# qimao7213/SInDSLAM

Measured on AMD Instinct MI355X. Metric: DynaDetect+ORB frame-pairs/sec at 640x480; mask IoU vs CPU ref, higher is better.
Workload: dtype f32

## Files before the change

include/sind_hip.h:

```cpp
#ifndef SIND_HIP_H
#define SIND_HIP_H
#include <stddef.h>
#include <stdint.h>
#ifdef __cplusplus
extern "C" {
#endif

#define SIND_OK 0
#define SIND_E_ARG (-1)
#define SIND_E_HIP (-2)
#define SIND_E_ALLOC (-3)
#define SIND_E_STATE (-4)
#define SIND_E_CAPACITY (-5)

const char* sind_last_error(void);
int sind_device_count(int* count);

typedef struct sind_flow sind_flow;
int sind_flow_create(int fw, int fh, int max_batch, int device, sind_flow** out);
int sind_flow_destroy(sind_flow* f);
int sind_flow_levels(sind_flow* f, int* widths, int* heights, int cap);
int sind_flow_deepflow(sind_flow* f, const uint8_t* i0, const uint8_t* i1, int B, float* u, float* v);
int sind_flow_refine(sind_flow* f, const uint8_t* i0, const uint8_t* i1, int B, float* u, float* v);
int sind_flow_varref_f32(sind_flow* f, const float* i0, const float* i1, int w, int h, int B, float* u, float* v,
                         int fixed_point_iters, int sor_iters, float alpha, float delta, float gamma, float omega);
int sind_flow_deepflow_dev(sind_flow* f, const uint8_t* i0, const uint8_t* i1, int B, float* u, float* v);
int sind_flow_refine_dev(sind_flow* f, const uint8_t* i0, const uint8_t* i1, int B, float* u, float* v);
int sind_flow_sync(sind_flow* f);
int sind_flow_set_max_levels(sind_flow* f, int n);
int sind_flow_set_coarse_chain(sind_flow* f, int on);
int sind_flow_set_latency_tiles(sind_flow* f, int on);
int sind_flow_set_level_up(sind_flow* f, int on);
int sind_flow_set_sor(sind_flow* f, int mode, int fuse, int tile_w);
int sind_flow_set_sor_tiled(sind_flow* f, int mode, int fuse, int tile_w, int tile_h);
int sind_flow_set_solver_workgroups(sind_flow* f, int cap);
int sind_flow_set_wave_solver(sind_flow* f, int on, int target_items, int bands);
int sind_flow_wave_layout(int w, int h, int B, int target_items, int bands, int out[4]);
int sind_flow_sor_plan(int mode, int fuse, int tile_w, int tile_h, int wave, int stream_min_b, int latency_tiles, int coarse_chain, int w, int h, int B, int total, int* out, int cap);
int sind_flow_set_coef_kernel(sind_flow* f, int variant);
int sind_flow_timer_begin(sind_flow* f);
int sind_flow_timer_end(sind_flow* f, float* milliseconds);

typedef struct sind_orb sind_orb;
typedef struct sind_keypoint { float x, y, size, angle, response; int octave, class_id; } sind_keypoint;
int sind_orb_create(int nfeatures, float scale_factor, int nlevels, int ini_th_fast, int min_th_fast, int device, sind_orb** out);
int sind_orb_destroy(sind_orb* o);
int sind_orb_reserve(sind_orb* o, int width, int height, int max_batch);
int sind_orb_extract(sind_orb* o, const uint8_t* gray, int width, int height, int stride, const uint8_t* mask_or_null, int mask_stride,
                     sind_keypoint* kps, int cap, int* n, uint8_t* desc );
int sind_orb_extract_batch(sind_orb* o, const uint8_t* gray, int width, int height, int B, const uint8_t* masks_or_null,
                           sind_keypoint* kps, int cap, int* n, uint8_t* desc);
int sind_orb_tables(sind_orb* o, float* scale, float* inv_scale, float* sigma2, float* inv_sigma2, int* features_per_level, int* umax16);
int sind_orb_pyramid(sind_orb* o, int frame, int level, uint8_t* out, int* w, int* h);
int sind_orb_debug_fast(sind_orb* o, int frame, int level, float* xyr, int cap);
int sind_orb_debug_selected(sind_orb* o, int frame, sind_keypoint* kps, int cap, uint8_t* desc);
int sind_orb_debug_blurred(sind_orb* o, int frame, int level, uint8_t* out, int* w, int* h);

typedef struct sind_dyna sind_dyna;
int sind_dyna_create(int width, int height, float fx, float fy, float cx, float cy, float depth_scale, int device, sind_dyna** out);
int sind_dyna_destroy(sind_dyna* d);
int sind_dyna_set_flow_max_levels(sind_dyna* d, int n);
int sind_dyna_timing(sind_dyna* d, double ms12[12], int reset);
int sind_dyna_timing_fine(sind_dyna* d, double ms40[40], int reset);
int sind_dyna_set_debug(sind_dyna* d, int on);
int sind_dyna_set_overlap(sind_dyna* d, int on);
int sind_dyna_prime(sind_dyna* d, const uint8_t* bgr_last, const uint8_t* bgr_lastlast, int stride);
int sind_dyna_detect(sind_dyna* d, const uint8_t* bgr, int bgr_stride, const uint16_t* depth, int depth_stride,
                     uint8_t* dyna_out, uint8_t* label_out, int n_img);
int sind_dyna_dilate15(sind_dyna* d, uint8_t* dyna_inout);
int sind_dyna_debug(sind_dyna* d, float* flow_deep, float* flow_refined, float* flow_full, double* H9, float* thr5, int* hist256,
                    uint8_t* mask_low, uint8_t* mask_high, uint8_t* kmeans_label, float* centers36, uint8_t* occ1, uint8_t* occ2,
                    uint8_t* total_area, uint8_t* grad_edge, uint8_t* plane_contours, int* info3);

int sind_debug_seqsum(const float* x, int n, int device, float* out);
int sind_debug_set_kmeans_fused_max(int n);
int sind_debug_set_kmeans_fused_min_batch(int b);
int sind_debug_coef_math_scan(int device, int exp_lo, int exp_hi, const float numer[3], unsigned long long out[2]);
int sind_debug_rcp_scan(int device, int exp_lo, int exp_hi, unsigned long long out[3]);
int sind_debug_div_scan(int device, unsigned long long counts[3], int* max_exp, unsigned long long by_exp[124]);

int sind_debug_flow_thresholds(const int* hist, int n, int width, int height, int variant, int device, int* res, double* mu1);
int sind_debug_large_motion(const float* u, const float* v, int B, int fw, int fh, int W, int H, int device, int* flags, int* hist, float* maxflow, int* end);
int sind_debug_flow_masks_batch(const float* u, const float* v, const double* homographies, int n, int width, int height, int device,
                                uint8_t* low_batch, uint8_t* high_batch, int* res_batch, uint8_t* low_frame, uint8_t* high_frame, int* res_frame);
int sind_debug_flow_masks_stage(const float* u, const float* v, const double* homographies, int n, int width, int height, int device,
                                uint8_t* low_batch, uint8_t* high_batch, int* res_batch, uint8_t* low_frame, uint8_t* high_frame, int* res_frame,
                                int byte_offset, float* mag_batch, uint8_t* magu8_batch, float* mag_frame, uint8_t* magu8_frame);

int sind_debug_peac_grow(const uint16_t* depth, int n, int width, int height, float fx, float fy, float cx, float cy, float depth_scale, int device,
                         int8_t* member_gpu, int8_t* member_host, uint8_t* pair_gpu, uint8_t* pair_host, int* status);

int sind_debug_depth_front(const uint16_t* depth, int n, int width, int height, float depth_scale, int device,
                           uint16_t* filt, unsigned* maxima, uint8_t* edge_pre, uint8_t* edge, uint8_t* total_area, uint8_t* depth_n);

int sind_debug_dilate_planes(const unsigned long long* planes, int nplanes, int width, int height, int n, int device, unsigned long long* out);
int sind_debug_rag_batch(const unsigned long long* planes, const int* pieces, const uint8_t* occ2, const uint8_t* depth_n, int n, int width, int height, int device,
                         int* out_batch, int* out_frame);

typedef struct sind_pipe sind_pipe;
typedef struct sind_pipe_config {
    int width, height; float fx, fy, cx, cy, depth_scale;
    int nfeatures; float scale_factor; int nlevels, ini_th_fast, min_th_fast;
    int orb_gray_rgb_order;
    int streams, frames_per_step, device;
    int host_threads;
    int flow_max_levels;
    int flow_slices;
    int flow_opts_off;
} sind_pipe_config;
int sind_pipe_create(const sind_pipe_config* cfg, sind_pipe** out);
int sind_pipe_destroy(sind_pipe* p);
int sind_pipe_prime(sind_pipe* p, int stream, const uint8_t* bgr_last, const uint8_t* bgr_lastlast);
int sind_pipe_process(sind_pipe* p, const uint8_t* bgr, const uint16_t* depth, uint8_t* dyna, uint8_t* label, uint8_t* mask_dilated,
                      sind_keypoint* kps, int cap, int* nkp, uint8_t* desc);
int sind_pipe_process_dev(sind_pipe* p, const uint8_t* bgr_dev, const uint16_t* depth_dev, uint8_t* dyna, uint8_t* label,
                          uint8_t* mask_dilated, sind_keypoint* kps, int cap, int* nkp, uint8_t* desc);
int sind_pipe_submit_dev(sind_pipe* p, const uint8_t* bgr_dev, const uint16_t* depth_dev, uint8_t* dyna, uint8_t* label, uint8_t* mask_dilated,
                         sind_keypoint* kps, int cap, int* nkp, uint8_t* desc, int* have_output);
int sind_pipe_flush(sind_pipe* p, uint8_t* dyna, uint8_t* label, uint8_t* mask_dilated, sind_keypoint* kps, int cap, int* nkp, uint8_t* desc,
                    int* have_output);
// ... 393 lines not shown
```

sindslam_amd/csrc/capi_flow.cpp:

```cpp
#include "../../include/sind_hip.h"
#include <cstring>
#include "flow.hpp"

struct sind_flow {
    int device = 0; hipStream_t stream = nullptr; sind::FlowEngine eng;
    DevBuf<uint8_t> g0, g1; DevBuf<float> u, v, f0, f1;
    hipEvent_t ev0 = nullptr, ev1 = nullptr;
};

extern "C" {

int sind_flow_set_max_levels(sind_flow* f, int n) { if (!f || n < 0) return SIND_E_ARG; f->eng.max_levels = n; return SIND_OK; }
int sind_flow_set_coarse_chain(sind_flow* f, int on) { if (!f) return SIND_E_ARG; f->eng.solver.coarse_chain = on != 0; return SIND_OK; }
int sind_flow_set_level_up(sind_flow* f, int on) { if (!f) return SIND_E_ARG; f->eng.solver.level_up = on != 0; return SIND_OK; }
int sind_flow_set_latency_tiles(sind_flow* f, int on) { if (!f) return SIND_E_ARG; f->eng.solver.latency_tiles = on != 0; return SIND_OK; }
int sind_device_count(int* count) { if (!count) return SIND_E_ARG; HIP_TRY(hipGetDeviceCount(count)); return SIND_OK; }

int sind_flow_create(int fw, int fh, int max_batch, int device, sind_flow** out) {
    if (!out || fw < 32 || fh < 32 || max_batch < 1) { sind_set_error("sind_flow_create: bad arguments"); return SIND_E_ARG; }
    HIP_TRY(hipSetDevice(device));
    sind_flow* f = new sind_flow(); f->device = device;
    HIP_TRY(hipStreamCreateWithFlags(&f->stream, hipStreamNonBlocking));
    HIP_TRY(hipEventCreate(&f->ev0)); HIP_TRY(hipEventCreate(&f->ev1));
    int r = f->eng.init(fw, fh, max_batch, f->stream);
// ... 138 lines not shown
        flags[b] = sind::large_motion_decision(m, h_hist.data() + (size_t)b * 256, W, H, end ? end + 2 * b : nullptr) ? 1 : 0;
        if (maxflow) maxflow[b] = m;
    }
    if (hist) std::copy(h_hist.begin(), h_hist.end(), hist);
    return SIND_OK;
}
int sind_debug_flow_masks_batch(const float* u, const float* v, const double* hm, int n, int width, int height, int device,
                                uint8_t* low_batch, uint8_t* high_batch, int* res_batch, uint8_t* low_frame, uint8_t* high_frame, int* res_frame) {
    return sind_debug_flow_masks_stage(u, v, hm, n, width, height, device, low_batch, high_batch, res_batch, low_frame, high_frame, res_frame, 0, nullptr, nullptr, nullptr, nullptr);
}
int sind_debug_flow_masks_stage(const float* u, const float* v, const double* hm, int n, int width, int height, int device,
                                uint8_t* low_batch, uint8_t* high_batch, int* res_batch, uint8_t* low_frame, uint8_t* high_frame, int* res_frame,
                                int byte_offset, float* mag_batch, uint8_t* magu8_batch, float* mag_frame, uint8_t* magu8_frame) {
    if (!u || !v || !hm || !low_batch || !high_batch || !res_batch || !low_frame || !high_frame || !res_frame || n < 1 || n > 64 || width < 64 || width % 64 != 0 || height < 1 || height > 4096 || width > 4096 ||
        byte_offset < 0 || byte_offset > 15) {
        sind_set_error("sind_debug_flow_masks_batch: bad arguments (1..64 frames, width a multiple of 64, byte offset 0..15)"); return SIND_E_ARG;
    }
    HIP_TRY(hipSetDevice(device));
    const size_t np = (size_t)width * height, words = np / 64, slot = sind::flow_mask_slot_words(width, height), res_off = (2 * np + byte_offset + 15) / 16 * 16;
    DevBuf<float> du, dv, dmag; DevBuf<uint8_t> dq, dqf, dmask; DevBuf<int> dh; DevBuf<unsigned long long> dout; DevBuf<sind::FlowMaskRec> drec;
    SIND_TRY(dqf.alloc(np + 16));
    SIND_TRY(du.alloc(np * n)); SIND_TRY(dv.alloc(np * n)); SIND_TRY(dmag.alloc(np * n)); SIND_TRY(dq.alloc(np * n)); SIND_TRY(dh.alloc((size_t)264 * n)); SIND_TRY(dout.alloc(slot * n)); SIND_TRY(drec.alloc(n));
    SIND_TRY(dmask.alloc(res_off + 1088));
    HIP_TRY(hipMemcpy(du.p, u, np * n * sizeof(float), hipMemcpyHostToDevice)); HIP_TRY(hipMemcpy(dv.p, v, np * n * sizeof(float), hipMemcpyHostToDevice));
    HIP_TRY(hipMemset(dh.p, 0, (size_t)264 * n * sizeof(int))); HIP_TRY(hipMemset(dout.p, 0, slot * n * 8));
    std::vector<sind::FlowMaskRec> recs(n);
    for (int i = 0; i < n; i++) { sind::FlowMaskRec& R = recs[i]; R.U = du.p + np * i; R.V = dv.p + np * i; std::copy(hm + 9 * i, hm + 9 * i + 9, R.H);
                                  R.mag = dmag.p + np * i; R.magu8 = dq.p + np * i; R.hist = dh.p + (size_t)264 * i; R.out = dout.p + slot * i; }
    HIP_TRY(hipMemcpy(drec.p, recs.data(), n * sizeof(sind::FlowMaskRec), hipMemcpyHostToDevice));
    SIND_TRY(sind::launch_flow_masks_frames(nullptr, drec.p, recs.data(), n, n, width, height));
    HIP_TRY(hipDeviceSynchronize());
    std::vector<unsigned long long> out(slot * n);
    HIP_TRY(hipMemcpy(out.data(), dout.p, out.size() * 8, hipMemcpyDeviceToHost));
    for (int i = 0; i < n; i++) {
        const unsigned long long* o = out.data() + slot * i;
        for (size_t k = 0; k < np; k++) { low_batch[np * i + k] = ((o[k >> 6] >> (k & 63)) & 1) ? 128 : 0; high_batch[np * i + k] = ((o[words + (k >> 6)] >> (k & 63)) & 1) ? 255 : 0; }
        std::memcpy(res_batch + (size_t)261 * i, o + 2 * words, 261 * sizeof(int));
    }
    if (mag_batch) HIP_TRY(hipMemcpy(mag_batch, dmag.p, np * n * sizeof(float), hipMemcpyDeviceToHost));
    if (magu8_batch) HIP_TRY(hipMemcpy(magu8_batch, dq.p, np * n, hipMemcpyDeviceToHost));
    uint8_t* q = dqf.p + byte_offset; uint8_t* low = dmask.p + byte_offset; uint8_t* high = low + np;
    for (int i = 0; i < n; i++) {
        int* res = reinterpret_cast<int*>(dmask.p + res_off);
        SIND_TRY(sind::launch_residual(nullptr, du.p + np * i, dv.p + np * i, hm + 9 * i, dmag.p, reinterpret_cast<unsigned*>(dh.p + 256), dh.p, q, width, height, false));
        SIND_TRY(sind::launch_flow_thresholds_and_masks(nullptr, dh.p, width, height, res, q, low, high));
        HIP_TRY(hipDeviceSynchronize());
        HIP_TRY(hipMemcpy(low_frame + np * i, low, np, hipMemcpyDeviceToHost)); HIP_TRY(hipMemcpy(high_frame + np * i, high, np, hipMemcpyDeviceToHost));
        HIP_TRY(hipMemcpy(res_frame + (size_t)261 * i, res, 261 * sizeof(int), hipMemcpyDeviceToHost));
        if (mag_frame) HIP_TRY(hipMemcpy(mag_frame + np * i, dmag.p, np * sizeof(float), hipMemcpyDeviceToHost));
        if (magu8_frame) HIP_TRY(hipMemcpy(magu8_frame + np * i, q, np, hipMemcpyDeviceToHost));
    }
    return SIND_OK;
}
static bool sor_tiled_ok(int mode, int fuse, int tile_w, int tile_h) {
    const int nt = tile_w * tile_h / 8;
    return (mode == 0 || mode == 4 || mode == 5 || mode == 6) && fuse >= 1 && fuse <= 12 && tile_w >= 16 && tile_w % 8 == 0 && tile_h >= 8 && tile_h % 2 == 0 && nt % 128 == 0 && nt <= 1024 &&
           4 * fuse < tile_w && 4 * fuse < tile_h;
}
int sind_flow_set_sor_tiled(sind_flow* f, int mode, int fuse, int tile_w, int tile_h) {
    if (!f) { sind_set_error("sind_flow_set_sor_tiled: null handle"); return SIND_E_ARG; }
    if (!sor_tiled_ok(mode, fuse, tile_w, tile_h)) { sind_set_error("sind_flow_set_sor_tiled: bad arguments (mode %d, fuse %d, tile %d x %d)", mode, fuse, tile_w, tile_h); return SIND_E_ARG; }
    sind::SolverCfg& C = f->eng.solver; C.mode = mode; C.fuse = fuse; C.tile_w = tile_w; C.tile_h = tile_h; return SIND_OK;
}
int sind_flow_sor_plan(int mode, int fuse, int tile_w, int tile_h, int wave, int stream_min_b, int latency_tiles, int coarse_chain, int w, int h, int B, int total, int* out, int cap) {
    if (!out || cap < 2 || w < 1 || h < 1 || B < 1 || total < 1 || stream_min_b < 1 || !sor_tiled_ok(mode, fuse, tile_w, tile_h)) { sind_set_error("sind_flow_sor_plan: bad arguments"); return SIND_E_ARG; }
    sind::SolverCfg C; C.mode = mode; C.fuse = fuse; C.tile_w = tile_w; C.tile_h = tile_h; C.wave = wave ? 1 : 0; C.stream_min_b = stream_min_b; C.latency_tiles = latency_tiles != 0; C.coarse_chain = coarse_chain != 0;
    sind::SorPlan plan;
    SIND_TRY(sind::sor_plan(w, h, B, total, sind::VarParams().epsilon, C, &plan));
    const int n = (int)plan.iters.size();
    if (cap < 2 + n) { sind_set_error("sind_flow_sor_plan: %d launches, room for %d", n, cap - 2); return SIND_E_ARG; }
    out[0] = (int)plan.kernel; out[1] = n; std::copy(plan.iters.begin(), plan.iters.end(), out + 2);
    return SIND_OK;
}
int sind_flow_set_solver_workgroups(sind_flow* f, int cap) { if (!f || cap < 0) return SIND_E_ARG; f->eng.solver.stream_wg_cap = cap; return SIND_OK; }
int sind_flow_set_wave_solver(sind_flow* f, int on, int target_items, int bands) {
    if (!f || target_items < 0 || bands < 0 || on < 0 || on > 4) return SIND_E_ARG;
    if (on > 1) f->eng.solver.wave_prefetch = std::min(on - 1, 3);
    f->eng.solver.wave = on ? 1 : 0; f->eng.solver.wave_items = target_items > 0 ? target_items : sind::SolverCfg().wave_items; f->eng.solver.wave_bands = bands; return SIND_OK;
}
int sind_flow_wave_layout(int w, int h, int B, int target_items, int bands, int out[4]) {
    if (w < 1 || h < 1 || B < 1 || target_items < 0 || bands < 0 || !out) return SIND_E_ARG;
    sind::sor_wave_layout(w, h, B, target_items > 0 ? target_items : sind::SolverCfg().wave_items, bands, &out[0], &out[1], &out[2], &out[3]); return SIND_OK;
}
int sind_flow_set_coef_kernel(sind_flow* f, int variant) { if (!f || variant < 0 || variant > 3) return SIND_E_ARG; f->eng.solver.coef_kernel = variant == 3 ? 1 : variant; f->eng.solver.coef_xcd = variant == 3 ? 0 : 1; return SIND_OK; }
int sind_flow_set_sor(sind_flow* f, int mode, int fuse, int tile_w) {
    if (tile_w != 64 && tile_w != 128) { sind_set_error("sind_flow_set_sor: bad arguments"); return SIND_E_ARG; }
    return sind_flow_set_sor_tiled(f, mode, fuse, tile_w, 64);
}
int sind_flow_sync(sind_flow* f) { if (!f) return SIND_E_ARG; HIP_TRY(hipStreamSynchronize(f->stream)); return SIND_OK; }
int sind_flow_timer_begin(sind_flow* f) { if (!f) return SIND_E_ARG; HIP_TRY(hipEventRecord(f->ev0, f->stream)); return SIND_OK; }
int sind_flow_timer_end(sind_flow* f, float* ms) {
    if (!f || !ms) return SIND_E_ARG;
    HIP_TRY(hipEventRecord(f->ev1, f->stream)); HIP_TRY(hipEventSynchronize(f->ev1)); HIP_TRY(hipEventElapsedTime(ms, f->ev0, f->ev1));
    return SIND_OK;
}

}
```

sindslam_amd/csrc/flow.hpp:

```cpp
#pragma once
#include "common.hpp"

namespace sind {

struct VarParams {
    int fixedPointIterations = 5, sorIterations = 5;
    float alpha = 20.0f, delta = 5.0f, gamma = 10.0f, omega = 1.6f, zeta = 0.1f, epsilon = 0.001f;
};
struct HMat { double h[9]; };
struct FlowMaskRec { const float* U; const float* V; double H[9]; float* mag; uint8_t* magu8; int* hist; unsigned long long* out; };

struct FlowPlanes {
    float *avg, *Iz;
    float *A11, *A12, *A22, *b1, *b2, *wgt;
    float *Wu, *Wv, *dWu, *dWv, *tWu, *tWv;
    float *dWu2, *dWv2;
};

struct SorTimer {
    std::vector<hipEvent_t> ev; std::vector<char> kind; size_t used = 0; bool enabled = false;
    double alg_bytes = 0, alg_bytes_other = 0; long long launches = 0, launches_other = 0;
    void begin(hipStream_t s) { if (!enabled) return; if (used + 2 > ev.size()) { hipEvent_t a, b; (void)hipEventCreate(&a); (void)hipEventCreate(&b); ev.push_back(a); ev.push_back(b); kind.push_back(0); } (void)hipEventRecord(ev[used], s); }
    void end(hipStream_t s, long long n_launches, double bytes, int k = 0) {
        if (!enabled) return;
        (void)hipEventRecord(ev[used + 1], s); kind[used / 2] = (char)k; used += 2;
        if (k == 0) { launches += n_launches; alg_bytes += bytes; } else { launches_other += n_launches; alg_bytes_other += bytes; }
    }
    void reset() { used = 0; alg_bytes = alg_bytes_other = 0; launches = launches_other = 0; }
    double collect_ms(int k = 0) { double t = 0; for (size_t i = 0; i + 1 < used; i += 2) { if (kind[i / 2] != k) continue; float ms = 0; if (hipEventElapsedTime(&ms, ev[i], ev[i + 1]) == hipSuccess) t += ms; } return t; }
    void intervals(hipEvent_t base, std::vector<std::pair<double, double>>& out, int k = 0) { for (size_t i = 0; i + 1 < used; i += 2) { if (kind[i / 2] != k) continue; float a = 0, b = 0; if (hipEventElapsedTime(&a, base, ev[i]) == hipSuccess && hipEventElapsedTime(&b, base, ev[i + 1]) == hipSuccess) out.emplace_back(a, b); } }
    ~SorTimer() { for (hipEvent_t e : ev) (void)hipEventDestroy(e); }
};

int launch_gather_frames(hipStream_t s, const uint8_t* pool, const int* idx_host, int B, uint8_t* out, size_t frame_bytes);
int launch_u8_to_f32_blur3(hipStream_t s, const uint8_t* src, float* dst, int w, int h, int B, float k0, float k1, bool blur);
int launch_resize_f32_pair(hipStream_t s, const float* srcA, float* dstA, const float* srcB, float* dstB, int sw, int sh, int dw, int dh, int B, float post, bool has_post);
int launch_pyramid_tail(hipStream_t s, float* pyrA, float* pyrB, const std::vector<std::pair<int, int>>& levels, const std::vector<size_t>& level_off, int first, int last, int B);
int launch_resize_f32(hipStream_t s, const float* src, float* dst, int sw, int sh, int dw, int dh, int B, float post, bool has_post);
int launch_resize_u8(hipStream_t s, const uint8_t* src, uint8_t* dst, int sw, int sh, int dw, int dh, int B, int s_stride, int d_stride, size_t s_img, size_t d_img, int d_group = 0, int d_skip = 0);
int launch_roll_history(hipStream_t s, uint8_t* pool, int S, int T, size_t frame_bytes);
int launch_bgr2gray(hipStream_t s, const uint8_t* bgr, uint8_t* gray, size_t npix, bool swap_rb);
int debug_rcp_scan(hipStream_t s, int exp_lo, int exp_hi, unsigned long long* out_dev);
int debug_div_scan(hipStream_t s, unsigned long long* out_dev);
int debug_coef_math_scan(hipStream_t s, int exp_lo, int exp_hi, const float numer[3], unsigned long long* out_dev);
struct SolverCfg {
    int mode = 4;
    int fuse = 5;
    int tile_w = 64, tile_h = 64;
    int stream_min_b = 80;
    int stream_wg_cap = 0;
    int wave = 1;
    int wave_items = 1024;
    int wave_bands = 0;
    int wave_prefetch = 2;
    int coef_kernel = 1;
    int coef_xcd = 1;
    bool coarse_chain = true;
    bool latency_tiles = true;
    bool level_up = true;
};
enum SorKernel { SOR_COARSE_CHAIN = 0, SOR_COLOR = 1, SOR_LATENCY_TILES = 2, SOR_ONE_WORKGROUP = 3, SOR_WAVE = 4, SOR_STREAM = 5, SOR_FUSED_TILES = 6 };
struct SorPlan { SorKernel kernel = SOR_COLOR; std::vector<int> iters; };
static inline int sor_timer_kind(SorKernel k) { return k == SOR_WAVE || k == SOR_STREAM ? 0 : 1; }
int sor_plan(int w, int h, int B, int total, float epsilon, const SolverCfg& C, SorPlan* plan);
bool chain_takes_level(int w, int h, float epsilon, const SolverCfg& C);
int sor_iterations(hipStream_t s, FlowPlanes& P, int w, int h, int B, float omega, const SorPlan& plan, const SolverCfg& C, long long* nlaunch);
int varref_level(hipStream_t s, FlowPlanes& P, const float* I0, const float* I1, int w, int h, int B, const VarParams& V, SorTimer* timer, const SolverCfg& C,
                 bool have_buffers = false, bool leave_increment = false);
int launch_level_up(hipStream_t s, FlowPlanes& P, int sw, int sh, const float* I0_next, const float* I1_next, int dw, int dh, int B, float post);
int coarse_level_P(int w, int h);
int launch_sor_tile(hipStream_t s, FlowPlanes& P, int w, int h, int B, int iters, float omega);
int launch_sor_wave(hipStream_t s, FlowPlanes& P, int w, int h, int B, float omega, int target_items, int force_bands, int prefetch);
void sor_wave_layout(int w, int h, int B, int target_items, int force_bands, int* strips, int* IW, int* bands, int* BH);
int sor_tile_count(int w, int h, int iters);
int launch_sor_stream(hipStream_t s, FlowPlanes& P, int w, int h, int B, float omega, int wg_cap);
bool sor_stream_fits(int h, int total);
int launch_coarse_chain(hipStream_t s, FlowPlanes& Pl, const float* pyr0, const float* pyr1, const std::vector<std::pair<int, int>>& levels, const std::vector<size_t>& level_off,
                        int first, int last, int B, const VarParams& V, bool init_zero, bool upsample_last, float post, float* out_u, float* out_v);
int launch_mag_stats(hipStream_t s, const float* u, const float* v, float* mag, unsigned* maxbits, int* hist, uint8_t* out_u8, int n, int B);
bool large_motion_decision(float maxFlow, const int* hist256, int W, int H, int* end2 = nullptr);
int launch_residual(hipStream_t s, const float* u, const float* v, const double H[9], float* mag, unsigned* maxbits, int* hist, uint8_t* magu8, int w, int h, bool already_zero = false);
int launch_flow_thresholds_and_masks(hipStream_t s, int* hist, int W, int H, int* res, const uint8_t* magu8, uint8_t* low, uint8_t* high);
static inline size_t flow_mask_slot_words(int W, int H) { return (2 * ((size_t)W * H / 64) + (261 * sizeof(int) + 7) / 8 + 1) / 2 * 2; }
int launch_flow_masks_frames(hipStream_t s, const FlowMaskRec* recs_dev, const FlowMaskRec* recs_host, int n, int capacity, int W, int H);
int debug_flow_thresholds(hipStream_t s, int* hist, int n, int W, int H, int variant, int* res, double* mu1);
int launch_gather_grid(hipStream_t s, const float* u, const float* v, float* out, int w, int h, int step, int B = 1);
int launch_scale2(hipStream_t s, float* a, float* b, float sc, size_t n);

class FlowEngine {
public:
    int fw = 0, fh = 0, maxB = 0;
    hipStream_t stream = nullptr;
    std::vector<std::pair<int, int>> levels;
    std::vector<size_t> level_off;
    size_t pyr_pixels = 0;
    int init(int fw, int fh, int maxB, hipStream_t s);
    int deepflow(const uint8_t* g0, const uint8_t* g1, int B, float* u, float* v);
    int refine(const uint8_t* g0, const uint8_t* g1, int B, float* u, float* v);
    int varref_f32(const float* I0, const float* I1, int w, int h, int B, float* u, float* v, const VarParams& V);
    FlowPlanes planes{};
    SorTimer sor_timer;
    int max_levels = 0;
    int launch_ahead = 3;
    SolverCfg solver;
    ~FlowEngine() { for (hipEvent_t e : level_done) (void)hipEventDestroy(e); }
private:
    DevBuf<float> plane_store, pyr0, pyr1;
    std::vector<hipEvent_t> level_done;
    float* level_ptr(DevBuf<float>& pyr, int l, int B) { return pyr.p + level_off[l] * (size_t)B; }
};

}
```

sindslam_amd/csrc/flow_sor.hip:

```cpp
#include "flow_dev.hpp"

namespace sind {

__global__ void k_sor_color(int w, int h, float omega, int color, const float* __restrict__ A11, const float* __restrict__ A12,
                            const float* __restrict__ A22, const float* __restrict__ B1, const float* __restrict__ B2,
                            const float* __restrict__ Wgt, float* __restrict__ dWu, float* __restrict__ dWv) {
    const int k = blockIdx.x * blockDim.x + threadIdx.x, y = blockIdx.y, b = blockIdx.z;
    const int x = 2 * k + ((y + color) & 1);
    if (x >= w) return;
    const size_t base = (size_t)b * w * h; const int i = y * w + x;
    const float* Wg = Wgt + base; float* U = dWu + base; float* V = dWv + base;
    const float wp = Wg[i];
    const float wl = x > 0 ? Wg[i - 1] : 0.f, wu = y > 0 ? Wg[i - w] : 0.f;
    const float ul = x > 0 ? U[i - 1] : 0.f, vl = x > 0 ? V[i - 1] : 0.f;
    const float ur = x < w - 1 ? U[i + 1] : 0.f, vr = x < w - 1 ? V[i + 1] : 0.f;
    const float uu = y > 0 ? U[i - w] : 0.f, vu = y > 0 ? V[i - w] : 0.f;
    const float ud = y < h - 1 ? U[i + w] : 0.f, vd = y < h - 1 ? V[i + w] : 0.f;
    const float sigmaU = wl * ul + wp * ur + wu * uu + wp * ud;
    const float sigmaV = wl * vl + wp * vr + wu * vu + wp * vd;
    float du = U[i], dv = V[i];
    const float a12 = A12[base + i];
    du += omega * ((sigmaU + B1[base + i] - dv * a12) / A11[base + i] - du);
    dv += omega * ((sigmaV + B2[base + i] - du * a12) / A22[base + i] - dv);
    U[i] = du; V[i] = dv;
// ... 147 lines not shown
static int sor_fused_attr() {
    static SindPerDeviceInit attr_init;
    HIP_TRY(attr_init.run([] {
        hipError_t attr_rc = hipSuccess;
        const void* fs[] = {(const void*)k_sor_fused<1024, 4, 0, 0>, (const void*)k_sor_fused<512, 2, 0, 0>, (const void*)k_sor_fused<512, 4, 64, 64>};
        for (const void* f : fs) if (attr_rc == hipSuccess) attr_rc = hipFuncSetAttribute(f, hipFuncAttributeMaxDynamicSharedMemorySize, 150 * 1024);
        return attr_rc;
    }));
    return SIND_OK;
}
static int launch_sor_color(hipStream_t s, FlowPlanes& P, int w, int h, int B, float omega) {
    const dim3 gs(divup(divup(w, 2), 64), h, B), bs(64);
    hipLaunchKernelGGL(k_sor_color, gs, bs, 0, s, w, h, omega, 0, P.A11, P.A12, P.A22, P.b1, P.b2, P.wgt, P.dWu, P.dWv);
    hipLaunchKernelGGL(k_sor_color, gs, bs, 0, s, w, h, omega, 1, P.A11, P.A12, P.A22, P.b1, P.b2, P.wgt, P.dWu, P.dWv);
    return SIND_OK;
}
static int launch_sor_fused_level(hipStream_t s, FlowPlanes& P, int w, int h, int B, int iters, float omega) {
    const int EW = (w + SOR_PX - 1) / SOR_PX * SOR_PX, EH = h, nt = sor_fused_threads(EW, EH);
    SIND_TRY(sor_fused_attr());
    auto kern1 = nt <= 512 ? k_sor_fused<512, 2, 0, 0> : k_sor_fused<1024, 4, 0, 0>;
    hipLaunchKernelGGL(kern1, dim3(1, B), dim3(nt), sor_fused_lds(EW, nt), s, w, h, EW, EH, EW, EH, 0, 0, 1, iters, 0, omega, P.A11, P.A12, P.A22, P.b1, P.b2, P.wgt,
                       P.dWu, P.dWv, P.dWu, P.dWv);
    return SIND_OK;
}
static int launch_sor_fused_tiles(hipStream_t s, FlowPlanes& P, int w, int h, int B, int k, float omega, const SolverCfg& C) {
    const int EW = C.tile_w, EH = C.tile_h, nt = sor_fused_threads(EW, EH);
    SIND_TRY(sor_fused_attr());
    const bool t64 = EW == 64 && EH == 64 && nt == 512;
    auto kern = t64 ? k_sor_fused<512, 4, 64, 64> : k_sor_fused<1024, 4, 0, 0>;
    const int halo = 2 * k, halo_x = halo, IW = EW - 2 * halo_x, IH = EH - 2 * halo;
    const int ntx = divup(w, IW), nty = divup(h, IH);
    hipLaunchKernelGGL(kern, dim3(ntx * nty, B), dim3(nt), sor_fused_lds(EW, nt), s, w, h, EW, EH, IW, IH, halo_x, halo, ntx, k, 1, omega, P.A11, P.A12, P.A22, P.b1, P.b2,
                       P.wgt, P.dWu, P.dWv, P.dWu2, P.dWv2);
    std::swap(P.dWu, P.dWu2); std::swap(P.dWv, P.dWv2);
    return SIND_OK;
}

static std::vector<int> sor_latency_plan(int w, int h, int B, int total) {
    const int slots = 256;
    for (int n = 1; n <= total; n++) {
        const int base = total / n, rem = total % n, kmax = base + (rem ? 1 : 0);
        if (kmax > 13) continue;
        if ((long long)sor_tile_count(w, h, kmax) * B > slots) { if (kmax <= 5) break; continue; }
        std::vector<int> plan((size_t)n, base);
        for (int i = 0; i < rem; i++) plan[(size_t)i]++;
        return plan;
    }
    return {};
}
bool chain_takes_level(int w, int h, float epsilon, const SolverCfg& C) { return C.coarse_chain && epsilon >= 1e-12f && coarse_level_P(w, h) != 0; }
int sor_plan(int w, int h, int B, int total, float epsilon, const SolverCfg& C, SorPlan* plan) {
    auto is = [&](SorKernel k, std::vector<int> iters) { plan->kernel = k; plan->iters = std::move(iters); return SIND_OK; };
    total = std::max(total, 0);
    if (C.mode == 0) return is(SOR_COLOR, std::vector<int>((size_t)total, 1));
    if (chain_takes_level(w, h, epsilon, C)) return is(SOR_COARSE_CHAIN, {total});
    const int EWw = (w + SOR_PX - 1) / SOR_PX * SOR_PX, nt1 = sor_fused_threads(EWw, h);
    if (C.latency_tiles && C.mode == 4) {
        std::vector<int> lat = sor_latency_plan(w, h, B, total);
        if (!lat.empty() && !(lat.size() > 1 && nt1 <= 512)) return is(SOR_LATENCY_TILES, std::move(lat));
    }
    if (nt1 <= SOR_NT) {
        const size_t shm = sor_fused_lds(EWw, nt1);
        if (shm > 150 * 1024) { sind_set_error("sor_iterations: a %d x %d level needs %zu bytes of LDS", w, h, shm); return SIND_E_ARG; }
        return is(SOR_ONE_WORKGROUP, {total});
    }
    const bool large = C.mode == 4 && B >= C.stream_min_b;
    if (total % 5 == 0 && (C.mode == 6 || (large && C.wave))) return is(SOR_WAVE, std::vector<int>((size_t)(total / 5), 5));
    if (sor_stream_fits(h, total) && (C.mode == 5 || large)) return is(SOR_STREAM, std::vector<int>((size_t)(total / 5), 5));
    const int EW = C.tile_w, EH = C.tile_h, nt = sor_fused_threads(EW, EH);
    if (nt > SOR_NT || 2 * 2 * C.fuse >= std::min(EW, EH)) { sind_set_error("sor_iterations: tile %d x %d / %d fused iterations not supported", EW, EH, C.fuse); return SIND_E_ARG; }
    const size_t shm = sor_fused_lds(EW, nt);
    if (shm > 150 * 1024) { sind_set_error("sor_iterations: %d x %d tiles need %zu bytes of LDS", EW, EH, shm); return SIND_E_ARG; }
    std::vector<int> tiles;
    for (int done = 0; done < total; done += tiles.back()) tiles.push_back(std::min(C.fuse, total - done));
    return is(SOR_FUSED_TILES, std::move(tiles));
}

int sor_iterations(hipStream_t s, FlowPlanes& P, int w, int h, int B, float omega, const SorPlan& plan, const SolverCfg& C, long long* nlaunch) {
    for (int k : plan.iters) {
        switch (plan.kernel) {
            case SOR_COLOR:         SIND_TRY(launch_sor_color(s, P, w, h, B, omega)); *nlaunch += 1; break;
            case SOR_LATENCY_TILES: SIND_TRY(launch_sor_tile(s, P, w, h, B, k, omega)); break;
            case SOR_ONE_WORKGROUP: SIND_TRY(launch_sor_fused_level(s, P, w, h, B, k, omega)); break;
            case SOR_WAVE:          SIND_TRY(launch_sor_wave(s, P, w, h, B, omega, C.wave_items, C.wave_bands, C.wave_prefetch)); break;
            case SOR_STREAM:        SIND_TRY(launch_sor_stream(s, P, w, h, B, omega, C.stream_wg_cap)); break;
            case SOR_FUSED_TILES:   SIND_TRY(launch_sor_fused_tiles(s, P, w, h, B, k, omega, C)); break;
            default: sind_set_error("sor_iterations: the coarse chain solves its levels itself"); return SIND_E_ARG;
        }
        *nlaunch += 1;
    }
    return SIND_OK;
}

}
```

sindslam_amd/csrc/flow_wave.hip:

```cpp
#include "flow_dev.hpp"

namespace sind {

#define SWV_NS 10
#define SWV_NW 12
#define SWV_ROWF (2 * 3 * 64)
#define SWV_HALO 10

struct SwvRow { float a11[2], a22[2], r11[2], r22[2], wp[2], du[2], dv[2]; };
typedef unsigned swv_u2 __attribute__((ext_vector_type(2)));

template <int I, bool IEEE>
__device__ __forceinline__ void swv_update(SwvRow& R, const SwvRow& U, const SwvRow& D, float a12, float b1, float b2, float omega, int& lo) {
    float lu, lv, ru, rv;
    if (I == 0) { lu = lane_prev(R.wp[1] * R.du[1]); lv = lane_prev(R.wp[1] * R.dv[1]); ru = R.wp[0] * R.du[1]; rv = R.wp[0] * R.dv[1]; }
    else        { lu = R.wp[0] * R.du[0]; lv = R.wp[0] * R.dv[0]; ru = R.wp[1] * lane_next(R.du[0]); rv = R.wp[1] * lane_next(R.dv[0]); }
    const float sigmaU = lu + ru + U.wp[I] * U.du[I] + R.wp[I] * D.du[I];
    const float sigmaV = lv + rv + U.wp[I] * U.dv[I] + R.wp[I] * D.dv[I];
    float nu = R.du[I], nv = R.dv[I];
    if (IEEE) sor_update_ieee(nu, nv, sigmaU + b1, sigmaV + b2, a12, R.a11[I], R.r11[I], R.a22[I], R.r22[I], omega);
    else sor_update_short(nu, nv, sigmaU + b1, sigmaV + b2, a12, R.a11[I], R.r11[I], R.a22[I], R.r22[I], omega, lo);
    R.du[I] = nu; R.dv[I] = nv;
}

extern __shared__ float swv_lds[];
struct SwvFlight { swv_u2 a11, a12, a22, b1, b2, w, u, v; };
struct SwvCtx {
    __amdgpu_buffer_rsrc_t pA11, pA12, pA22, pB1, pB2, pW, pU, pV, oU, oV;
    float* lbase; float omega; unsigned xoff, row_bytes; int ys; unsigned nrows; int by0, by1; bool in0, in1, keep0, keep1;
};
typedef decltype(__builtin_amdgcn_raw_buffer_load_b64(__amdgpu_buffer_rsrc_t(), 0, 0, 0)) swv_b64;

struct SwvRec { float a12, b1, b2; };
template <int K, int S>
__device__ __forceinline__ SwvRec swv_record(const SwvCtx& C) {
    constexpr int NW = SWV_NW, sl = (K - S + 2 * NW) % NW;
    const float* lrow = C.lbase + sl * SWV_ROWF + (K & 1) * 192;
    return SwvRec{lrow[0], lrow[64], lrow[128]};
}
template <int K, int S, bool IEEE>
__device__ __forceinline__ void swv_stages(SwvRow (&win)[SWV_NW], const SwvCtx& C, int t, SwvRec rec, int& lo) {
    if constexpr (S < SWV_NS) {
        const int y = t - S;
        SwvRec next{};
        if constexpr (S + 1 < SWV_NS) next = swv_record<K, S + 1>(C);
        if ((unsigned)(y - C.ys) < C.nrows) {
            constexpr int NW = SWV_NW, sl = (K - S + 2 * NW) % NW, up = (sl + NW - 1) % NW, dn = (sl + 1) % NW;
#ifdef SWV_SKIP
            if (S < SWV_SKIP)
#endif
            swv_update<K & 1, IEEE>(win[sl], win[up], win[dn], rec.a12, rec.b1, rec.b2, C.omega, lo);
            if (S == SWV_NS - 1 && y >= C.by0 && y < C.by1) {
                const unsigned ro = (unsigned)y * C.row_bytes;
                const SwvRow& R = win[sl];
                if (C.keep1) {
                    __builtin_amdgcn_raw_buffer_store_b64(__builtin_bit_cast(swv_b64, swv_u2{__float_as_uint(R.du[0]), __float_as_uint(R.du[1])}), C.oU, C.xoff, ro, 0);
                    __builtin_amdgcn_raw_buffer_store_b64(__builtin_bit_cast(swv_b64, swv_u2{__float_as_uint(R.dv[0]), __float_as_uint(R.dv[1])}), C.oV, C.xoff, ro, 0);
                } else if (C.keep0) {
                    __builtin_amdgcn_raw_buffer_store_b32(__float_as_uint(R.du[0]), C.oU, C.xoff, ro, 0);
                    __builtin_amdgcn_raw_buffer_store_b32(__float_as_uint(R.dv[0]), C.oV, C.xoff, ro, 0);
                }
            }
        }
        __builtin_amdgcn_sched_barrier(0);
        swv_stages<K, S + 1, IEEE>(win, C, t, next, lo);
    }
}
template <int K, int PF, bool IEEE>
__device__ __forceinline__ void swv_steps(SwvRow (&win)[SWV_NW], SwvFlight (&FL)[PF], const SwvCtx& C, int t0, int& lo) {
    if constexpr (K < SWV_NW) {
        const int t = t0 + K;
        const SwvRec rec0 = swv_record<K, 0>(C);
        SwvFlight& F = FL[K % PF];
        {
            SwvRow& N = win[(K + 1) % SWV_NW];
            const bool ok = (unsigned)(t + 1 - C.ys) < C.nrows;
            const bool m0 = ok && C.in0, m1 = ok && C.in1;
            N.du[0] = m0 ? __uint_as_float(F.u.x) : 0.f; N.du[1] = m1 ? __uint_as_float(F.u.y) : 0.f;
            N.dv[0] = m0 ? __uint_as_float(F.v.x) : 0.f; N.dv[1] = m1 ? __uint_as_float(F.v.y) : 0.f;
            N.a11[0] = __uint_as_float(F.a11.x); N.a11[1] = __uint_as_float(F.a11.y); N.a22[0] = __uint_as_float(F.a22.x); N.a22[1] = __uint_as_float(F.a22.y);
            N.wp[0] = __uint_as_float(F.w.x); N.wp[1] = __uint_as_float(F.w.y);
            const float q0 = sor_rcp(N.a11[0]), q1 = sor_rcp(N.a11[1]), q2 = sor_rcp(N.a22[0]), q3 = sor_rcp(N.a22[1]);
            N.r11[0] = m0 ? q0 : 0.f; N.r11[1] = m1 ? q1 : 0.f; N.r22[0] = m0 ? q2 : 0.f; N.r22[1] = m1 ? q3 : 0.f;
            float* lr = C.lbase + ((K + 1) % SWV_NW) * SWV_ROWF;
            lr[0] = __uint_as_float(F.a12.x); lr[64] = __uint_as_float(F.b1.x); lr[128] = __uint_as_float(F.b2.x);
            lr[192] = __uint_as_float(F.a12.y); lr[256] = __uint_as_float(F.b1.y); lr[320] = __uint_as_float(F.b2.y);
        }
        if ((unsigned)(t + 1 + PF - C.ys) < C.nrows && C.in0) {
#ifdef SWV_ROWFIX
            const unsigned ro = (unsigned)C.ys * C.row_bytes;
#else
            const unsigned ro = (unsigned)(t + 1 + PF) * C.row_bytes;
#endif
            auto ld = [&](const __amdgpu_buffer_rsrc_t& r) { return __builtin_bit_cast(swv_u2, __builtin_amdgcn_raw_buffer_load_b64(r, C.xoff, ro, 0)); };
            F.u = ld(C.pU); F.v = ld(C.pV); F.a11 = ld(C.pA11); F.a22 = ld(C.pA22); F.w = ld(C.pW); F.a12 = ld(C.pA12); F.b1 = ld(C.pB1); F.b2 = ld(C.pB2);
        }
        __builtin_amdgcn_sched_barrier(0);
        swv_stages<K, 0, IEEE>(win, C, t, rec0, lo);
        swv_steps<K + 1, PF, IEEE>(win, FL, C, t0, lo);
    }
}

template <int PF>
__global__ void __launch_bounds__(64) __attribute__((amdgpu_waves_per_eu(2, 2)))
k_sor_wave(int strips, int bands, int items, int w, int h, int IW, int BH, float omega, const float* __restrict__ gA11, const float* __restrict__ gA12, const float* __restrict__ gA22,
           const float* __restrict__ gB1, const float* __restrict__ gB2, const float* __restrict__ gW, const float* __restrict__ gU, const float* __restrict__ gV,
           float* __restrict__ gUo, float* __restrict__ gVo) {
    const int lane = threadIdx.x;
    const int per_xcd = (int)gridDim.x >> 3, item = ((int)blockIdx.x & 7) * per_xcd + ((int)blockIdx.x >> 3);
    if (item >= items) return;
    const int strip = item % strips, rest = item / strips, band = rest % bands, image = rest / bands;
    const int ix0 = strip * IW, ix1 = min(ix0 + IW, w), ex0 = max(ix0 - SWV_HALO, 0);
    const int by0 = band * BH, by1 = min(by0 + BH, h), ys = max(by0 - SWV_HALO, 0), ye = min(by1 + SWV_HALO, h);
    const unsigned nrows = (unsigned)(ye - ys);
    const int x0 = ex0 + 2 * lane;
    const bool in0 = x0 < w, in1 = x0 + 1 < w;
    const bool keep0 = x0 >= ix0 && x0 < ix1, keep1 = x0 + 1 >= ix0 && x0 + 1 < ix1;
    const size_t base = (size_t)image * w * h;
    const unsigned plane_bytes = (unsigned)w * (unsigned)h * 4u;
    auto rs = [&](const float* plane) { return __builtin_amdgcn_make_buffer_rsrc((void*)(plane + base), 0, plane_bytes, 0x00020000); };
    const SwvCtx C{rs(gA11), rs(gA12), rs(gA22), rs(gB1), rs(gB2), rs(gW), rs(gU), rs(gV), rs(gUo), rs(gVo),
                   swv_lds + lane, omega, (unsigned)x0 * 4u, (unsigned)w * 4u, ys, nrows, by0, by1, in0, in1, keep0, keep1};
    const int Tb = (ys - 1 - PF) & ~1, Tend = ye + SWV_NS - 1;
    int lo = 0;
    {
        SwvRow win[SWV_NW] = {};
        SwvFlight FL[PF] = {};
        for (int t0 = Tb; t0 < Tend; t0 += SWV_NW) swv_steps<0, PF, false>(win, FL, C, t0, lo);
    }
    if (__builtin_amdgcn_ballot_w64(lo < DIV_TINY_FREXP) != 0) {
        SwvRow win[SWV_NW] = {};
        SwvFlight FL[PF] = {};
        for (int t0 = Tb; t0 < Tend; t0 += SWV_NW) swv_steps<0, PF, true>(win, FL, C, t0, lo);
    }
}

void sor_wave_layout(int w, int h, int B, int target_items, int force_bands, int* strips, int* IW, int* bands, int* BH) {
    int n = 1, iw = (w + 1) & ~1;
    if (w > 128) { for (n = 2;; n++) { iw = (divup(w, n) + 1) & ~1; if (iw + (n == 2 ? SWV_HALO : 2 * SWV_HALO) <= 128) break; } }
    int nb = force_bands > 0 ? force_bands : (int)std::min<long long>(std::max(1, h / 40), std::max<long long>(1, divup(target_items, n * std::max(B, 1))));
    nb = std::max(1, std::min(nb, h));
    const int bh = divup(h, nb);
    nb = divup(h, bh);
    *strips = n; *IW = iw; *bands = nb; *BH = bh;
}

int launch_sor_wave(hipStream_t s, FlowPlanes& P, int w, int h, int B, float omega, int target_items, int force_bands, int prefetch) {
    int strips, IW, bands, BH;
    sor_wave_layout(w, h, B, target_items, force_bands, &strips, &IW, &bands, &BH);
    if ((long long)w * h > (1ll << 28)) { sind_set_error("launch_sor_wave: %d x %d level", w, h); return SIND_E_ARG; }
    const size_t shm = (size_t)SWV_NW * SWV_ROWF * sizeof(float);
    const int items = strips * bands * B;
    auto kern = prefetch <= 1 ? k_sor_wave<1> : prefetch == 2 ? k_sor_wave<2> : k_sor_wave<3>;
    hipLaunchKernelGGL(kern, dim3((unsigned)(divup(items, 8) * 8)), dim3(64), shm, s, strips, bands, items, w, h, IW, BH, omega, P.A11, P.A12, P.A22, P.b1, P.b2, P.wgt, P.dWu, P.dWv, P.dWu2, P.dWv2);
    std::swap(P.dWu, P.dWu2); std::swap(P.dWv, P.dWv2);
    return SIND_OK;
}

}
```

sindslam_amd/flow.py:

```python
from __future__ import annotations

import ctypes as C

import numpy as np

from ._lib import check, lib, ptr


class FlowStage:
    def __init__(self, fw: int = 384, fh: int = 288, max_batch: int = 8, device: int = 0):
        self.fw, self.fh, self.max_batch = fw, fh, max_batch
        h = C.c_void_p()
        check(lib().sind_flow_create(fw, fh, max_batch, device, C.byref(h)), "sind_flow_create")
        self._h = h

    def set_max_levels(self, n: int):
        check(lib().sind_flow_set_max_levels(self._h, int(n)), "sind_flow_set_max_levels")

    def set_sor_variant(self, mode: int = 4, fuse: int = 5, tile_w: int = 64, tile_h: int = 64):
        check(lib().sind_flow_set_sor_tiled(self._h, mode, fuse, tile_w, tile_h), "sind_flow_set_sor_tiled")

    def set_solver_workgroups(self, cap: int):
        check(lib().sind_flow_set_solver_workgroups(self._h, int(cap)), "sind_flow_set_solver_workgroups")

    def set_wave_solver(self, on: bool = True, target_items: int = 0, bands: int = 0):
        check(lib().sind_flow_set_wave_solver(self._h, 1 if on else 0, int(target_items), int(bands)), "sind_flow_set_wave_solver")

    def set_coef_kernel(self, variant: int):
        check(lib().sind_flow_set_coef_kernel(self._h, int(variant)), "sind_flow_set_coef_kernel")

    def set_coarse_chain(self, on: bool):
        check(lib().sind_flow_set_coarse_chain(self._h, 1 if on else 0), "sind_flow_set_coarse_chain")

    def set_level_up(self, on: bool):
        check(lib().sind_flow_set_level_up(self._h, 1 if on else 0), "sind_flow_set_level_up")

    def set_latency_tiles(self, on: bool):
        check(lib().sind_flow_set_latency_tiles(self._h, 1 if on else 0), "sind_flow_set_latency_tiles")

    def close(self):
        if getattr(self, "_h", None):
            lib().sind_flow_destroy(self._h); self._h = None

    __del__ = close

    def levels(self):
        ws = np.zeros(256, np.int32); hs = np.zeros(256, np.int32)
        n = check(lib().sind_flow_levels(self._h, ptr(ws), ptr(hs), 256)); return list(zip(ws[:n].tolist(), hs[:n].tolist()))

    def deepflow(self, i0: np.ndarray, i1: np.ndarray):
        i0 = np.ascontiguousarray(i0, np.uint8); i1 = np.ascontiguousarray(i1, np.uint8)
        B = i0.shape[0]; u = np.empty(i0.shape, np.float32); v = np.empty(i0.shape, np.float32)
        check(lib().sind_flow_deepflow(self._h, ptr(i0), ptr(i1), B, ptr(u), ptr(v)), "sind_flow_deepflow"); return u, v

    def refine(self, i0, i1, u, v):
        i0 = np.ascontiguousarray(i0, np.uint8); i1 = np.ascontiguousarray(i1, np.uint8)
        u = np.array(u, np.float32, copy=True, order="C"); v = np.array(v, np.float32, copy=True, order="C")
        check(lib().sind_flow_refine(self._h, ptr(i0), ptr(i1), i0.shape[0], ptr(u), ptr(v)), "sind_flow_refine"); return u, v

    def varref_f32(self, i0, i1, u, v, fp_iters=5, sor_iters=5, alpha=20.0, delta=5.0, gamma=10.0, omega=1.6):
        i0 = np.ascontiguousarray(i0, np.float32); i1 = np.ascontiguousarray(i1, np.float32)
        u = np.array(u, np.float32, copy=True, order="C"); v = np.array(v, np.float32, copy=True, order="C")
        B, h, w = i0.shape
        check(lib().sind_flow_varref_f32(self._h, ptr(i0), ptr(i1), w, h, B, ptr(u), ptr(v), fp_iters, sor_iters, C.c_float(alpha),
                                         C.c_float(delta), C.c_float(gamma), C.c_float(omega)), "sind_flow_varref_f32"); return u, v

    def deepflow_dev(self, i0_ptr: int, i1_ptr: int, B: int, u_ptr: int, v_ptr: int):
        check(lib().sind_flow_deepflow_dev(self._h, ptr(i0_ptr), ptr(i1_ptr), B, ptr(u_ptr), ptr(v_ptr)), "sind_flow_deepflow_dev")

    def refine_dev(self, i0_ptr, i1_ptr, B, u_ptr, v_ptr):
        check(lib().sind_flow_refine_dev(self._h, ptr(i0_ptr), ptr(i1_ptr), B, ptr(u_ptr), ptr(v_ptr)), "sind_flow_refine_dev")

    def sync(self):
        check(lib().sind_flow_sync(self._h), "sind_flow_sync")

    def timer_begin(self):
        check(lib().sind_flow_timer_begin(self._h))

    def timer_end(self) -> float:
        ms = C.c_float(); check(lib().sind_flow_timer_end(self._h, C.byref(ms))); return ms.value
```

Measured before the change: 1617.

## Pack several small-level images side by side in wave SOR strips

Result: faster. 1671 (median of 6 runs) (+3.4%).

```diff
diff --git a/include/sind_hip.h b/include/sind_hip.h
--- a/include/sind_hip.h
+++ b/include/sind_hip.h
@@ -36,6 +36,8 @@
 int sind_flow_set_solver_workgroups(sind_flow* f, int cap);
 int sind_flow_set_wave_solver(sind_flow* f, int on, int target_items, int bands);
 int sind_flow_wave_layout(int w, int h, int B, int target_items, int bands, int out[4]);
+int sind_flow_set_wave_pack(sind_flow* f, int group);
+int sind_flow_wave_pack_layout(int w, int h, int B, int target_items, int bands, int group, int out[6]);
 int sind_flow_sor_plan(int mode, int fuse, int tile_w, int tile_h, int wave, int stream_min_b, int latency_tiles, int coarse_chain, int w, int h, int B, int total, int* out, int cap);
 int sind_flow_set_coef_kernel(sind_flow* f, int variant);
 int sind_flow_timer_begin(sind_flow* f);
diff --git a/sindslam_amd/csrc/capi_flow.cpp b/sindslam_amd/csrc/capi_flow.cpp
--- a/sindslam_amd/csrc/capi_flow.cpp
+++ b/sindslam_amd/csrc/capi_flow.cpp
@@ -244,6 +244,12 @@
     if (w < 1 || h < 1 || B < 1 || target_items < 0 || bands < 0 || !out) return SIND_E_ARG;
     sind::sor_wave_layout(w, h, B, target_items > 0 ? target_items : sind::SolverCfg().wave_items, bands, &out[0], &out[1], &out[2], &out[3]); return SIND_OK;
 }
+int sind_flow_set_wave_pack(sind_flow* f, int group) { if (!f || group < 0) return SIND_E_ARG; f->eng.solver.wave_group = group; return SIND_OK; }
+int sind_flow_wave_pack_layout(int w, int h, int B, int target_items, int bands, int group, int out[6]) {
+    if (w < 1 || h < 1 || B < 1 || target_items < 0 || bands < 0 || group < 0 || !out) return SIND_E_ARG;
+    const sind::SorWavePack L = sind::sor_wave_pack_layout(w, h, B, target_items > 0 ? target_items : sind::SolverCfg().wave_items, bands, group);
+    out[0] = L.G; out[1] = L.Pw; out[2] = L.strips; out[3] = L.IW; out[4] = L.bands; out[5] = L.BH; return SIND_OK;
+}
 int sind_flow_set_coef_kernel(sind_flow* f, int variant) { if (!f || variant < 0 || variant > 3) return SIND_E_ARG; f->eng.solver.coef_kernel = variant == 3 ? 1 : variant; f->eng.solver.coef_xcd = variant == 3 ? 0 : 1; return SIND_OK; }
 int sind_flow_set_sor(sind_flow* f, int mode, int fuse, int tile_w) {
     if (tile_w != 64 && tile_w != 128) { sind_set_error("sind_flow_set_sor: bad arguments"); return SIND_E_ARG; }
diff --git a/sindslam_amd/csrc/flow.hpp b/sindslam_amd/csrc/flow.hpp
--- a/sindslam_amd/csrc/flow.hpp
+++ b/sindslam_amd/csrc/flow.hpp
@@ -53,6 +53,7 @@
     int wave_items = 1024;
     int wave_bands = 0;
     int wave_prefetch = 2;
+    int wave_group = 0;
     int coef_kernel = 1;
     int coef_xcd = 1;
     bool coarse_chain = true;
@@ -70,8 +71,10 @@
 int launch_level_up(hipStream_t s, FlowPlanes& P, int sw, int sh, const float* I0_next, const float* I1_next, int dw, int dh, int B, float post);
 int coarse_level_P(int w, int h);
 int launch_sor_tile(hipStream_t s, FlowPlanes& P, int w, int h, int B, int iters, float omega);
-int launch_sor_wave(hipStream_t s, FlowPlanes& P, int w, int h, int B, float omega, int target_items, int force_bands, int prefetch);
+int launch_sor_wave(hipStream_t s, FlowPlanes& P, int w, int h, int B, float omega, int target_items, int force_bands, int prefetch, int force_group);
 void sor_wave_layout(int w, int h, int B, int target_items, int force_bands, int* strips, int* IW, int* bands, int* BH);
+struct SorWavePack { int G, Pw, strips, IW, bands, BH; };
+SorWavePack sor_wave_pack_layout(int w, int h, int B, int target_items, int force_bands, int force_group);
 int sor_tile_count(int w, int h, int iters);
 int launch_sor_stream(hipStream_t s, FlowPlanes& P, int w, int h, int B, float omega, int wg_cap);
 bool sor_stream_fits(int h, int total);
diff --git a/sindslam_amd/csrc/flow_sor.hip b/sindslam_amd/csrc/flow_sor.hip
--- a/sindslam_amd/csrc/flow_sor.hip
+++ b/sindslam_amd/csrc/flow_sor.hip
@@ -253,7 +253,7 @@
             case SOR_COLOR:         SIND_TRY(launch_sor_color(s, P, w, h, B, omega)); *nlaunch += 1; break;
             case SOR_LATENCY_TILES: SIND_TRY(launch_sor_tile(s, P, w, h, B, k, omega)); break;
             case SOR_ONE_WORKGROUP: SIND_TRY(launch_sor_fused_level(s, P, w, h, B, k, omega)); break;
-            case SOR_WAVE:          SIND_TRY(launch_sor_wave(s, P, w, h, B, omega, C.wave_items, C.wave_bands, C.wave_prefetch)); break;
+            case SOR_WAVE:          SIND_TRY(launch_sor_wave(s, P, w, h, B, omega, C.wave_items, C.wave_bands, C.wave_prefetch, C.wave_group)); break;
             case SOR_STREAM:        SIND_TRY(launch_sor_stream(s, P, w, h, B, omega, C.stream_wg_cap)); break;
             case SOR_FUSED_TILES:   SIND_TRY(launch_sor_fused_tiles(s, P, w, h, B, k, omega, C)); break;
             default: sind_set_error("sor_iterations: the coarse chain solves its levels itself"); return SIND_E_ARG;
diff --git a/sindslam_amd/csrc/flow_wave.hip b/sindslam_amd/csrc/flow_wave.hip
--- a/sindslam_amd/csrc/flow_wave.hip
+++ b/sindslam_amd/csrc/flow_wave.hip
@@ -103,24 +103,30 @@
 
 template <int PF>
 __global__ void __launch_bounds__(64) __attribute__((amdgpu_waves_per_eu(2, 2)))
-k_sor_wave(int strips, int bands, int items, int w, int h, int IW, int BH, float omega, const float* __restrict__ gA11, const float* __restrict__ gA12, const float* __restrict__ gA22,
-           const float* __restrict__ gB1, const float* __restrict__ gB2, const float* __restrict__ gW, const float* __restrict__ gU, const float* __restrict__ gV,
+k_sor_wave(int strips, int bands, int items, int w, int h, int IW, int BH, int G, int Pw, int B, float omega, const float* __restrict__ gA11, const float* __restrict__ gA12,
+           const float* __restrict__ gA22, const float* __restrict__ gB1, const float* __restrict__ gB2, const float* __restrict__ gW, const float* __restrict__ gU, const float* __restrict__ gV,
            float* __restrict__ gUo, float* __restrict__ gVo) {
     const int lane = threadIdx.x;
     const int per_xcd = (int)gridDim.x >> 3, item = ((int)blockIdx.x & 7) * per_xcd + ((int)blockIdx.x >> 3);
     if (item >= items) return;
-    const int strip = item % strips, rest = item / strips, band = rest % bands, image = rest / bands;
-    const int ix0 = strip * IW, ix1 = min(ix0 + IW, w), ex0 = max(ix0 - SWV_HALO, 0);
+    const int strip = item % strips, rest = item / strips, band = rest % bands, group = rest / bands;
+    const int image0 = group * G, present = min(G, B - image0);
+    const int vw = (present - 1) * Pw + w;
+    const int ix0 = strip * IW, ix1 = min(ix0 + IW, vw), ex0 = max(ix0 - SWV_HALO, 0);
+    if (ix0 >= vw) return;
     const int by0 = band * BH, by1 = min(by0 + BH, h), ys = max(by0 - SWV_HALO, 0), ye = min(by1 + SWV_HALO, h);
     const unsigned nrows = (unsigned)(ye - ys);
-    const int x0 = ex0 + 2 * lane;
-    const bool in0 = x0 < w, in1 = x0 + 1 < w;
-    const bool keep0 = x0 >= ix0 && x0 < ix1, keep1 = x0 + 1 >= ix0 && x0 + 1 < ix1;
-    const size_t base = (size_t)image * w * h;
-    const unsigned plane_bytes = (unsigned)w * (unsigned)h * 4u;
-    auto rs = [&](const float* plane) { return __builtin_amdgcn_make_buffer_rsrc((void*)(plane + base), 0, plane_bytes, 0x00020000); };
+    const int xv = ex0 + 2 * lane, li = xv / Pw, x0 = xv - li * Pw;
+    int xa = li < present ? x0 : w, xk = (li < present && x0 < w) ? xv : -2;
+    asm volatile("" : "+v"(xa), "+v"(xk));
+    const bool in0 = xa < w, in1 = xa + 1 < w;
+    const bool keep0 = xk >= ix0 && xk < ix1, keep1 = in1 && xk + 1 >= ix0 && xk + 1 < ix1;
+    const size_t base = (size_t)image0 * w * h;
+    const unsigned plane = (unsigned)w * (unsigned)h, group_bytes = (unsigned)present * plane * 4u;
+    auto rs = [&](const float* p) { return __builtin_amdgcn_make_buffer_rsrc((void*)(p + base), 0, group_bytes, 0x00020000); };
+    const unsigned xoff = in0 ? ((unsigned)li * plane + (unsigned)x0) * 4u : 0u;
     const SwvCtx C{rs(gA11), rs(gA12), rs(gA22), rs(gB1), rs(gB2), rs(gW), rs(gU), rs(gV), rs(gUo), rs(gVo),
-                   swv_lds + lane, omega, (unsigned)x0 * 4u, (unsigned)w * 4u, ys, nrows, by0, by1, in0, in1, keep0, keep1};
+                   swv_lds + lane, omega, xoff, (unsigned)w * 4u, ys, nrows, by0, by1, in0, in1, keep0, keep1};
     const int Tb = (ys - 1 - PF) & ~1, Tend = ye + SWV_NS - 1;
     int lo = 0;
     {
@@ -135,24 +141,43 @@
     }
 }
 
+static void swv_strips(int W, int* strips, int* IW) {
+    int n = 1, iw = (W + 1) & ~1;
+    if (W > 128) { for (n = 2;; n++) { iw = (divup(W, n) + 1) & ~1; if (iw + (n == 2 ? SWV_HALO : 2 * SWV_HALO) <= 128) break; } }
+    *strips = n; *IW = iw;
+}
 void sor_wave_layout(int w, int h, int B, int target_items, int force_bands, int* strips, int* IW, int* bands, int* BH) {
-    int n = 1, iw = (w + 1) & ~1;
-    if (w > 128) { for (n = 2;; n++) { iw = (divup(w, n) + 1) & ~1; if (iw + (n == 2 ? SWV_HALO : 2 * SWV_HALO) <= 128) break; } }
+    int n, iw;
+    swv_strips(w, &n, &iw);
     int nb = force_bands > 0 ? force_bands : (int)std::min<long long>(std::max(1, h / 40), std::max<long long>(1, divup(target_items, n * std::max(B, 1))));
     nb = std::max(1, std::min(nb, h));
     const int bh = divup(h, nb);
     nb = divup(h, bh);
     *strips = n; *IW = iw; *bands = nb; *BH = bh;
 }
+SorWavePack sor_wave_pack_layout(int w, int h, int B, int target_items, int force_bands, int force_group) {
+    SorWavePack L{1, (w + 2) & ~1, 0, 0, 0, 0};
+    sor_wave_layout(w, h, B, target_items, force_bands, &L.strips, &L.IW, &L.bands, &L.BH);
+    const int gmax = (int)std::min<long long>(std::min(32, std::max(B, 1)), std::max<long long>(1, (1ll << 29) / ((long long)w * h)));
+    const int lo = force_group > 0 ? std::min(force_group, gmax) : 2, hi = force_group > 0 ? lo : gmax;
+    long long best = (long long)B * L.strips;
+    for (int G = std::max(lo, 2); G <= hi; G++) {
+        int n, iw;
+        swv_strips((G - 1) * L.Pw + w, &n, &iw);
+        const long long total = (long long)divup(B, G) * n;
+        if (force_group > 0 || total < best) { best = total; L.G = G; L.strips = n; L.IW = iw; }
+    }
+    return L;
+}
 
-int launch_sor_wave(hipStream_t s, FlowPlanes& P, int w, int h, int B, float omega, int target_items, int force_bands, int prefetch) {
-    int strips, IW, bands, BH;
-    sor_wave_layout(w, h, B, target_items, force_bands, &strips, &IW, &bands, &BH);
+int launch_sor_wave(hipStream_t s, FlowPlanes& P, int w, int h, int B, float omega, int target_items, int force_bands, int prefetch, int force_group) {
     if ((long long)w * h > (1ll << 28)) { sind_set_error("launch_sor_wave: %d x %d level", w, h); return SIND_E_ARG; }
+    const SorWavePack L = sor_wave_pack_layout(w, h, B, target_items, force_bands, force_group);
     const size_t shm = (size_t)SWV_NW * SWV_ROWF * sizeof(float);
-    const int items = strips * bands * B;
+    const int items = L.strips * L.bands * divup(B, L.G);
     auto kern = prefetch <= 1 ? k_sor_wave<1> : prefetch == 2 ? k_sor_wave<2> : k_sor_wave<3>;
-    hipLaunchKernelGGL(kern, dim3((unsigned)(divup(items, 8) * 8)), dim3(64), shm, s, strips, bands, items, w, h, IW, BH, omega, P.A11, P.A12, P.A22, P.b1, P.b2, P.wgt, P.dWu, P.dWv, P.dWu2, P.dWv2);
+    hipLaunchKernelGGL(kern, dim3((unsigned)(divup(items, 8) * 8)), dim3(64), shm, s, L.strips, L.bands, items, w, h, L.IW, L.BH, L.G, L.Pw, B, omega, P.A11, P.A12, P.A22, P.b1, P.b2, P.wgt,
+                       P.dWu, P.dWv, P.dWu2, P.dWv2);
     std::swap(P.dWu, P.dWu2); std::swap(P.dWv, P.dWv2);
     return SIND_OK;
 }
diff --git a/sindslam_amd/flow.py b/sindslam_amd/flow.py
--- a/sindslam_amd/flow.py
+++ b/sindslam_amd/flow.py
@@ -25,6 +25,9 @@
 
     def set_wave_solver(self, on: bool = True, target_items: int = 0, bands: int = 0):
         check(lib().sind_flow_set_wave_solver(self._h, 1 if on else 0, int(target_items), int(bands)), "sind_flow_set_wave_solver")
+
+    def set_wave_pack(self, group: int = 0):
+        check(lib().sind_flow_set_wave_pack(self._h, int(group)), "sind_flow_set_wave_pack")
 
     def set_coef_kernel(self, variant: int):
         check(lib().sind_flow_set_coef_kernel(self._h, int(variant)), "sind_flow_set_coef_kernel")
```
